# huangzh13/StyleGAN.pytorch

Measured on AMD Instinct MI355X. Metric: img/s full G+D train step, 1024x1024 depth-9 bf16, higher is better.
Workload: dtype bf16; 1 GPU; ffhq1024: StyleGAN 1024x1024, progressive depth index 8, logistic+R1, alpha 0.5, batch 4/GPU, global batch 4; global_batch=4, parallelism=dp1

## Files before the change

### include/sgx.h

```cpp
#ifndef SGX_H
#define SGX_H
#include <stddef.h>
#include <stdint.h>
#ifdef __cplusplus
extern "C" {
#endif

enum { SGX_F32 = 0, SGX_BF16 = 1 };
enum { SGX_ACT_NONE = 0, SGX_ACT_LRELU = 1, SGX_ACT_RELU = 2 };
enum { SGX_EINVAL = -1, SGX_EUNSUPPORTED = -2, SGX_EWORKSPACE = -3 };

int sgx_version(void);
const char* sgx_last_error(void);
int sgx_clear_error(void);
int sgx_stream_wait_stream(void* waiter, void* signaler);
int sgx_selftest_tr16(void* out256, void* stream);

int sgx_prof_start(int mode, int only_of);
int sgx_prof_count(void);
int sgx_prof_get(int i, char* name, int name_cap, float* ms, double* flops, double* bytes, char* desc, int desc_cap);

int sgx_conv3x3(const void* x, const void* w, const float* bias, void* y, int B, int H, int W, int Cin, int Cout,
                int act, const void* mask, int dtype, void* stream);
int sgx_conv4x4s2_down(const void* x, const void* w, const float* bias, void* y, int B, int H, int W, int Cin,
// ... 103 lines not shown
int sgx_rgbconv_pack(const float* w0, float s0, const float* wr, float sr, const float* br, float bscale, void* wf, void* wd, int C,
                     void* stream);
int sgx_rgbconv_fwd(const float* img, const void* wf, const float* b0, void* y, void* bits, int B, int H, int W, int C, int epi, int ones,
                    int dtype, void* stream);
int sgx_rgbconv_tune(int fwd_variant, int nit, int dbg);
int sgx_rgbconv_dgrad(const void* gz, const void* wd, float* gi, int B, int H, int W, int C, int dtype, void* stream);
size_t sgx_rgbconv_wgrad_ws_bytes(int B, int H, int W, int C);
int sgx_rgbconv_wgrad(const float* img, const void* gz, int ones, const float* w0, float s0, const float* wr, float sr, const float* br,
                      float bscale, float* dw0, float* db0, float* dwr, float* dbr, int acc, void* ws, size_t ws_bytes, int B, int H, int W,
                      int C, int dtype, void* stream);
int sgx_blur3x3_stats(const void* x, void* y, const float* bias, const float* noise, const float* nw, double* part,
                      size_t part_bytes, int B, int H, int W, int C, int act, int dtype, void* stream);
int sgx_gepi_bwd(const void* dy, const void* x, const float* bias, const float* noise, const float* nw,
                 const float* style, const float* mean, const float* rstd, void* dx, float* dstyle, float* dnw,
                 float* dbias, void* ws, size_t ws_bytes, int B, int HW, int C, int flags, int dtype, void* stream);

int sgx_pixelnorm_fwd(const float* x, float* y, int B, int C, void* stream);
int sgx_pixelnorm_bwd(const float* dy, const float* x, float* dx, int B, int C, void* stream);
int sgx_mbstd_fwd(const void* x, void* y, int B, int HW, int C, int Cpad, int dtype, void* stream);
int sgx_mbstd_bwd(const void* dy, const void* x, void* dx, int B, int HW, int C, int Cpad, int dtype, void* stream);
int sgx_mbstd_bwd2(const void* ggx, const void* dy, const void* x, void* ddy, void* gx, int B, int HW, int C, int Cpad,
                   int dtype, void* stream);
size_t sgx_sumsq_ws_bytes(void);
int sgx_sumsq_f32(const float* x, size_t n, void* ws, size_t ws_bytes, float* out, void* stream);
int sgx_scale_dev_f32(const float* x, const float* s, float alpha, float* out, size_t n, void* stream);
int sgx_logistic_loss(const float* fake, int n_fake, const float* real, int n_real, float scale, int generator, float* loss,
                      float* g_fake, float* g_real, void* stream);
size_t sgx_gemm_ws_bytes(int M, int N, int K);
int sgx_gemm_f32(const float* A, const float* Bm, float* C, int M, int N, int K, int ta, int tb, float alpha,
                 void* ws, size_t ws_bytes, void* stream);
// ... 34 lines not shown
```

### stylegan/pytorch_amd/Blocks.py

```python
import os

import torch
import torch.nn as nn

from . import functional as F
from .CustomLayers import (BlurLayer, EqualizedConv2d, EqualizedLinear, LayerEpilogue, StddevLayer, View, act_code, apply_act)
from .native import ACT_LRELU, ACT_NONE


FUSE_EPI_STATS = int(os.environ.get("SGX_FUSE_EPI_STATS", "2"))
FUSE_EPI_STATS_MIN = int(os.environ.get("SGX_FUSE_EPI_STATS_MIN", str(1 << 27)))


FUSE_BLUR_BWD = os.environ.get("SGX_FUSE_BLUR_BWD", "1") != "0"


def _lat(d, k):
    return d[k] if isinstance(d, (tuple, list)) else d[:, k]


class InputBlock(nn.Module):

    def __init__(self, nf, dlatent_size, const_input_layer, gain, use_wscale, use_noise, use_pixel_norm,
                 use_instance_norm, use_styles, activation_layer):
# ... 38 lines not shown
        self.conv0_up = EqualizedConv2d(in_channels, out_channels, kernel_size=3, gain=gain, use_wscale=use_wscale,
                                        intermediate=blur, upscale=True)
        self.epi1 = LayerEpilogue(out_channels, dlatent_size, use_wscale, use_noise, use_pixel_norm,
                                  use_instance_norm, use_styles, activation_layer)
        self.conv1 = EqualizedConv2d(out_channels, out_channels, kernel_size=3, gain=gain, use_wscale=use_wscale)
        self.epi2 = LayerEpilogue(out_channels, dlatent_size, use_wscale, use_noise, use_pixel_norm,
                                  use_instance_norm, use_styles, activation_layer)

    def forward_nhwc(self, x, dlatents_in_range, defer_epi2=False):
        up = self.conv0_up
        if (FUSE_EPI_STATS & 1) and self.epi1._fusable and up.intermediate is not None and up.intermediate._is_121:
            b, h, w, _ = x.shape
            nin = self.epi1.noise_inputs((b, 2 * h, 2 * w, up.weight.shape[0]), x.device)
            x, part = up.forward_nhwc(x, skip_bias=True, epi_stats=(up.scaled_bias(),) + nin)
            x = self.epi1.forward_nhwc(x, _lat(dlatents_in_range, 0), conv_bias=up.scaled_bias(), noise_in=nin, pre_stats=part)
        else:
            x = up.forward_nhwc(x, skip_bias=True)
            x = self.epi1.forward_nhwc(x, _lat(dlatents_in_range, 0), conv_bias=up.scaled_bias())
        defer_epi2 = defer_epi2 and self.epi2._fusable
        if (FUSE_EPI_STATS & 2) and self.epi2._fusable and x.numel() >= FUSE_EPI_STATS_MIN:
            nin = self.epi2.noise_inputs(x.shape, x.device)
            x, part = self.conv1.forward_nhwc(x, skip_bias=True, epi_stats=(self.conv1.scaled_bias(),) + nin)
            if defer_epi2:
                return x, (self.conv1.scaled_bias(), nin[0], nin[1], self.epi2._style(_lat(dlatents_in_range, 1)), part)
            return self.epi2.forward_nhwc(x, _lat(dlatents_in_range, 1), conv_bias=self.conv1.scaled_bias(), noise_in=nin, pre_stats=part)
        if defer_epi2:
            nin = self.epi2.noise_inputs(x.shape, x.device)
            x = self.conv1.forward_nhwc(x, skip_bias=True)
            return x, (self.conv1.scaled_bias(), nin[0], nin[1], self.epi2._style(_lat(dlatents_in_range, 1)), None)
        x = self.conv1.forward_nhwc(x, skip_bias=True)
# ... 94 lines not shown
```

### stylegan/pytorch_amd/CustomLayers.py

```python
import math

import numpy as np
import torch
import torch.nn as nn

from . import functional as F
from .native import ACT_LRELU, ACT_NONE, ACT_RELU, EPI_ACT, EPI_NORM

MBSTD_CPAD = 32


def act_code(activation_layer):
    if isinstance(activation_layer, nn.LeakyReLU) and abs(activation_layer.negative_slope - 0.2) < 1e-12:
        return ACT_LRELU
    if activation_layer is torch.relu or isinstance(activation_layer, nn.ReLU):
        return ACT_RELU
    raise NotImplementedError(f"activation {activation_layer!r}: the reference offers 'lrelu' (0.2) and 'relu'")


def apply_act(x, act):
    return F.call(F.BiasActFn, x, None, 1.0, act) if act else x


class PixelNormLayer(nn.Module):
# ... 144 lines not shown
        if bias:
            self.bias = nn.Parameter(torch.zeros(output_channels))
            self.b_mul = lrmul
        else:
            self.bias = None
            self.b_mul = 1
        self.intermediate = intermediate
        assert stride == 1

    def scaled_bias(self):
        if self.bias is None:
            return None
        return self.bias * self.b_mul if self.b_mul != 1 else self.bias

    def forward_nhwc(self, x, act=ACT_NONE, skip_bias=False, out_dtype=None, defer_act=False, x_masked=False, out_scale=1.0,
                     epi_stats=None, x_pre=None, sign_bits=False, x_pre_bits=None, fade=None):
        bias = None if skip_bias else self.scaled_bias()
        cin, cout = self.weight.shape[1], self.weight.shape[0]
        if self.kernel_size == 1:
            assert self.upscale is None and self.downscale is None and self.intermediate is None
            if cin == 3 and x.shape[3] == 3:
                if out_scale != 1.0:
                    y = F.call(F.RgbInFn, x.float(), self.weight, None if bias is None else bias * float(out_scale),
                               self.w_mul * float(out_scale), out_dtype or torch.float32)
                else:
                    y = F.call(F.RgbInFn, x.float(), self.weight, bias, self.w_mul, out_dtype or torch.float32)
            elif cin % 3 == 0 and cin > 3 and x.shape[3] == cin and cout != 3:
                y = None
                for k in range(0, cin, 3):
                    part = F.call(F.RgbInFn, x[..., k:k + 3].float().contiguous(), self.weight[:, k:k + 3].contiguous(),
                                  bias if k == 0 else None, self.w_mul, out_dtype or torch.float32)
# ... 7 lines not shown
        if epi_stats is not None:
            assert skip_bias and act == ACT_NONE and self.downscale is None
            ebias, noise, nw = epi_stats
            if self.upscale is not None:
                fused = min(x.shape[1], x.shape[2]) * 2 >= 128
                y = F.conv(x, self.weight, None, "U" if fused else "UF", self.w_mul)
                assert self.intermediate is not None and self.intermediate._is_121
                return F.call(F.BlurStatsFn, y, ebias, noise, nw)
            assert self.intermediate is None
            if F.conv_stats_nparts(x, self.weight.shape[0]) > 0:
                return F.conv(x, self.weight, None, "S", self.w_mul, ipad=x.shape[3], stats=(ebias, noise, nw))
            return F.conv(x, self.weight, None, "S", self.w_mul, ipad=x.shape[3]), None
        if self.upscale is not None:
            fused = min(x.shape[1], x.shape[2]) * 2 >= 128
            mode = "U" if fused else "UF"
            if (self.intermediate is not None and self.intermediate._is_121
                    and F.conv_blur_ok(x, self.weight.shape[0], mode, False)):
                y = F.call(F.ConvBlurFn, x, self.weight, mode, float(self.w_mul), int(self.weight.shape[1]), False, None)
            else:
                y = F.conv(x, self.weight, None, mode, self.w_mul)
                if self.intermediate is not None:
                    y = self.intermediate.forward_nhwc(y)
            if bias is not None or act:
                y = F.call(F.BiasActFn, y, bias, 1.0, act)
            return y
        if self.downscale is not None:
            assert self.intermediate is None
            if fade is not None:
                assert act == ACT_LRELU and not x_masked
                if x_pre is not None and getattr(x, "_sgx_pre_of", None) is not x_pre:
# ... 77 lines not shown
        self.top_epi = nn.Sequential(OrderedDict(layers))
        self.style_mod = StyleMod(dlatent_size, channels, use_wscale=use_wscale) if use_styles else None
        self._act = act_code(activation_layer)
        self._use = (bool(use_noise), bool(use_pixel_norm), bool(use_instance_norm), bool(use_styles))
        self._fusable = use_noise and use_instance_norm and use_styles and not use_pixel_norm and self._act == ACT_LRELU

    def _style(self, dlatents_in_slice):
        if isinstance(dlatents_in_slice, F.PreStyle):
            return dlatents_in_slice.style
        return self.style_mod.style(dlatents_in_slice)

    def noise_inputs(self, x_shape, device):
        noise_layer = self.top_epi.noise
        return noise_layer.sample(x_shape, device), noise_layer.weight

    def forward_nhwc(self, x, dlatents_in_slice, conv_bias=None, noise_in=None, pre_stats=None):
        use_noise, use_pixel_norm, use_instance_norm, use_styles = self._use
        noise = nw = None
        if noise_in is not None:
            noise, nw = noise_in
        elif use_noise:
            noise, nw = self.noise_inputs(x.shape, x.device)
        style = self._style(dlatents_in_slice) if use_styles else None
        if self._fusable:
            return F.call(F.GEpilogueFn, x, conv_bias, noise, nw, style, EPI_ACT | EPI_NORM, pre_stats)
        assert pre_stats is None
        lrelu = self._act == ACT_LRELU
        norm = EPI_NORM if use_instance_norm else 0
        if lrelu and not use_pixel_norm:
            return F.call(F.GEpilogueFn, x, conv_bias, noise, nw, style, EPI_ACT | norm)
        x = F.call(F.GEpilogueFn, x, conv_bias, noise, nw, None, EPI_ACT if lrelu else 0)
        if not lrelu:
            x = apply_act(x, self._act)
        if use_pixel_norm:
            shape, dt = x.shape, x.dtype
            x = F.call(F.PixelNormFn, x.reshape(-1, shape[3])).reshape(shape).to(dt)
        if norm or style is not None:
            x = F.call(F.GEpilogueFn, x, None, None, None, style, norm)
        return x

    def forward(self, x, dlatents_in_slice=None):
# ... 48 lines not shown
```

### stylegan/pytorch_amd/functional.py

```python
import contextlib
import functools
import os
import weakref

import numpy as np
import torch
from torch.autograd import Function
from torch.autograd.function import once_differentiable

from . import native as N

_DATA_GRAD_ONLY = 0


@contextlib.contextmanager
def data_grad_only():
    global _DATA_GRAD_ONLY
    _DATA_GRAD_ONLY += 1
    try:
        yield
    finally:
        _DATA_GRAD_ONLY -= 1


# ... 1545 lines not shown
        x, bias_c, noise, nw_c, style_c, mean, rstd = ctx.saved_tensors
        gy = _c(gy)
        B, H, W, C = x.shape
        dx = torch.empty_like(x)
        dstyle = torch.empty((B, 2 * C), dtype=torch.float32, device=x.device)
        dnw = torch.empty((C,), dtype=torch.float32, device=x.device)
        dbias = torch.empty((C,), dtype=torch.float32, device=x.device) if ctx.has_bias else None
        L = N.lib()
        ws = N.workspace(L.sgx_gepi_ws_bytes(B, H * W, C), x.device)
        N.check(L.sgx_gepi_bwd(N.ptr(gy), N.ptr(x), N.ptr(bias_c), N.ptr(noise), N.ptr(nw_c), N.ptr(style_c), N.ptr(mean), N.ptr(rstd),
                               N.ptr(dx), N.ptr(dstyle), N.ptr(dnw), N.ptr(dbias), N.ptr(ws), ws.numel(), B, H * W, C, ctx.flags,
                               N.dt(x), N.stream()), "sgx_gepi_bwd")
        return dx, dbias, None, dnw if ctx.has_noise else None, dstyle if ctx.has_style else None, None, None


FUSE_EPI_RGB = os.environ.get("SGX_FUSE_EPI_RGB", "1") != "0"


def epi_rgb_out_ok(C, dtype):
    ve = 4 if dtype == torch.float32 else 8
    if dtype not in (torch.float32, torch.bfloat16) or C % ve or C > 2048:
        return False
    lpp = min(C // ve, 16)
    return lpp & (lpp - 1) == 0


class EpiRgbOutFn(Function):

    @staticmethod
    def forward(ctx, y, ebias, noise, nw, style, weight, rbias, wscale, low, alpha, pre=None):
# ... 521 lines not shown
```

### stylegan/pytorch_amd/native.py

```python
import ctypes
import os
import subprocess
import threading

import torch

_HERE = os.path.dirname(os.path.abspath(__file__))
LIB_PATH = os.environ.get("SGX_HIP_LIB") or os.path.join(_HERE, "libsgx_hip.so")
CSRC = os.path.join(_HERE, "csrc")

F32, BF16 = 0, 1
ACT_NONE, ACT_LRELU, ACT_RELU = 0, 1, 2
EPI_ACT, EPI_NORM = 1, 2
PACK_S, PACK_D, PACK_U, PACK_UF = 0, 1, 2, 3

_lib = None
_lock = threading.Lock()

c_void_p, c_int, c_float, c_size_t = ctypes.c_void_p, ctypes.c_int, ctypes.c_float, ctypes.c_size_t
P, I, F, Z = c_void_p, c_int, c_float, c_size_t

SIGNATURES = {
    "sgx_version": (I, []),
    "sgx_last_error": (ctypes.c_char_p, []),
# ... 65 lines not shown
    "sgx_conv4x4s2_up_blur": (I, [P, P, P, P, I, I, I, I, I, I, P]),
    "sgx_conv4x4s2_up_blur_bits": (I, [P, P, P, P, I, I, I, I, I, I, P]),
    "sgx_pack_upblur": (I, [P, P, I, I, I, I, F, P]),
    "sgx_conv_upblur_ok": (I, [I, I, I, I, I, I]),
    "sgx_conv_upblur": (I, [P, P, P, P, I, I, I, I, I, I, P]),
    "sgx_rgbconv_ok": (I, [I, I, I, I, I]),
    "sgx_rgbconv_pack": (I, [P, F, P, F, P, F, P, P, I, P]),
    "sgx_rgbconv_fwd": (I, [P, P, P, P, P, I, I, I, I, I, I, I, P]),
    "sgx_rgbconv_tune": (I, [I, I, I]),
    "sgx_rgbconv_dgrad": (I, [P, P, P, I, I, I, I, I, P]),
    "sgx_rgbconv_wgrad_ws_bytes": (Z, [I, I, I, I]),
    "sgx_rgbconv_wgrad": (I, [P, P, I, P, F, P, F, P, F, P, P, P, P, I, P, Z, I, I, I, I, I, P]),
    "sgx_conv3x3_stats": (I, [P, P, P, P, P, P, P, Z, I, I, I, I, I, I, P]),
    "sgx_blur3x3_stats": (I, [P, P, P, P, P, P, Z, I, I, I, I, I, I, P]),
    "sgx_gepi_bwd": (I, [P, P, P, P, P, P, P, P, P, P, P, P, P, Z, I, I, I, I, I, P]),
    "sgx_pixelnorm_fwd": (I, [P, P, I, I, P]),
    "sgx_pixelnorm_bwd": (I, [P, P, P, I, I, P]),
    "sgx_mbstd_fwd": (I, [P, P, I, I, I, I, I, P]),
    "sgx_mbstd_bwd": (I, [P, P, P, I, I, I, I, I, P]),
    "sgx_mbstd_bwd2": (I, [P, P, P, P, P, I, I, I, I, I, P]),
    "sgx_sumsq_ws_bytes": (Z, []),
    "sgx_sumsq_f32": (I, [P, Z, P, Z, P, P]),
    "sgx_scale_dev_f32": (I, [P, P, F, P, Z, P]),
    "sgx_logistic_loss": (I, [P, I, P, I, F, I, P, P, P, P]),
    "sgx_gemm_ws_bytes": (Z, [I, I, I]),
    "sgx_gemm_f32": (I, [P, P, P, I, I, I, I, I, F, P, Z, P]),
    "sgx_linear_fwd": (I, [P, P, P, P, I, I, I, F, F, I, P]),
    "sgx_linear_bwd_data": (I, [P, P, P, P, I, I, I, F, P]),
    "sgx_linear_bwd_param": (I, [P, P, P, P, P, I, I, I, F, F, P]),
    "sgx_style_fwd": (I, [P, P, P, I, I, I, I, P]),
# ... 217 lines not shown
```

Baseline: 290.1 img/s.

## Fuse blur, noise, bias, lrelu, instance norm and style into single-pass generator layer kernel

Adds a fused generator-layer kernel (forward and backward) for small and mid-resolution layers. It keeps each per-channel-group image slice resident in registers or LDS, computes the instance-norm statistics in-block, and applies the epilogue without a second pass over memory. For upsample layers where the conv+blur fused path is unavailable, the blur is folded into the same kernel. The backward uses ticket-based last-block reduction for the noise-weight and bias gradients, which saves a separate finish launch but adds atomics and a persistent ticket buffer.

```diff
diff --git a/include/sgx.h b/include/sgx.h
--- a/include/sgx.h
+++ b/include/sgx.h
@@ -141,6 +141,12 @@
 int sgx_gepi_bwd(const void* dy, const void* x, const float* bias, const float* noise, const float* nw,
                  const float* style, const float* mean, const float* rstd, void* dx, float* dstyle, float* dnw,
                  float* dbias, void* ws, size_t ws_bytes, int B, int HW, int C, int flags, int dtype, void* stream);
+int sgx_glayer_ok(int B, int H, int W, int C, int flags, int dtype);
+int sgx_glayer_fwd(const void* x, int blur, const float* bias, const float* noise, const float* nw, const float* style, void* xb, void* y,
+                   float* mean, float* rstd, int B, int H, int W, int C, int flags, int dtype, void* stream);
+int sgx_glayer_bwd(const void* dy, const void* xb, int blur, const float* bias, const float* noise, const float* nw, const float* style,
+                   const float* mean, const float* rstd, void* dx, float* dstyle, float* dnw, float* dbias, double* part, int* tickets,
+                   int B, int H, int W, int C, int flags, int dtype, void* stream);
 
 int sgx_pixelnorm_fwd(const float* x, float* y, int B, int C, void* stream);
 int sgx_pixelnorm_bwd(const float* dy, const float* x, float* dx, int B, int C, void* stream);
diff --git a/stylegan/pytorch_amd/Blocks.py b/stylegan/pytorch_amd/Blocks.py
--- a/stylegan/pytorch_amd/Blocks.py
+++ b/stylegan/pytorch_amd/Blocks.py
@@ -76,6 +76,11 @@
             nin = self.epi1.noise_inputs((b, 2 * h, 2 * w, up.weight.shape[0]), x.device)
             x, part = up.forward_nhwc(x, skip_bias=True, epi_stats=(up.scaled_bias(),) + nin)
             x = self.epi1.forward_nhwc(x, _lat(dlatents_in_range, 0), conv_bias=up.scaled_bias(), noise_in=nin, pre_stats=part)
+        elif (up.intermediate is not None and up.intermediate._is_121
+              and self.epi1.glayer_takes((x.shape[0], 2 * x.shape[1], 2 * x.shape[2], up.weight.shape[0]), x.dtype)
+              and not F.conv_blur_ok(x, up.weight.shape[0], "U" if min(x.shape[1], x.shape[2]) * 2 >= 128 else "UF", False)):
+            x = up.forward_nhwc(x, skip_bias=True, skip_blur=True)
+            x = self.epi1.forward_nhwc(x, _lat(dlatents_in_range, 0), conv_bias=up.scaled_bias(), blur=True)
         else:
             x = up.forward_nhwc(x, skip_bias=True)
             x = self.epi1.forward_nhwc(x, _lat(dlatents_in_range, 0), conv_bias=up.scaled_bias())
diff --git a/stylegan/pytorch_amd/CustomLayers.py b/stylegan/pytorch_amd/CustomLayers.py
--- a/stylegan/pytorch_amd/CustomLayers.py
+++ b/stylegan/pytorch_amd/CustomLayers.py
@@ -182,7 +182,7 @@
         return self.bias * self.b_mul if self.b_mul != 1 else self.bias
 
     def forward_nhwc(self, x, act=ACT_NONE, skip_bias=False, out_dtype=None, defer_act=False, x_masked=False, out_scale=1.0,
-                     epi_stats=None, x_pre=None, sign_bits=False, x_pre_bits=None, fade=None):
+                     epi_stats=None, x_pre=None, sign_bits=False, x_pre_bits=None, fade=None, skip_blur=False):
         bias = None if skip_bias else self.scaled_bias()
         cin, cout = self.weight.shape[1], self.weight.shape[0]
         if self.kernel_size == 1:
@@ -220,6 +220,9 @@
         if self.upscale is not None:
             fused = min(x.shape[1], x.shape[2]) * 2 >= 128
             mode = "U" if fused else "UF"
+            if skip_blur:
+                assert skip_bias and not act and self.intermediate is not None and self.intermediate._is_121
+                return F.conv(x, self.weight, None, mode, self.w_mul)
             if (self.intermediate is not None and self.intermediate._is_121
                     and F.conv_blur_ok(x, self.weight.shape[0], mode, False)):
                 y = F.call(F.ConvBlurFn, x, self.weight, mode, float(self.w_mul), int(self.weight.shape[1]), False, None)
@@ -327,7 +330,10 @@
         noise_layer = self.top_epi.noise
         return noise_layer.sample(x_shape, device), noise_layer.weight
 
-    def forward_nhwc(self, x, dlatents_in_slice, conv_bias=None, noise_in=None, pre_stats=None):
+    def glayer_takes(self, x_shape, dtype):
+        return bool(self._fusable and F.glayer_ok(x_shape, dtype))
+
+    def forward_nhwc(self, x, dlatents_in_slice, conv_bias=None, noise_in=None, pre_stats=None, blur=False):
         use_noise, use_pixel_norm, use_instance_norm, use_styles = self._use
         noise = nw = None
         if noise_in is not None:
@@ -336,8 +342,11 @@
             noise, nw = self.noise_inputs(x.shape, x.device)
         style = self._style(dlatents_in_slice) if use_styles else None
         if self._fusable:
+            if pre_stats is None and F.glayer_ok(x.shape, x.dtype):
+                return F.call(F.GLayerFn, x, conv_bias, noise, nw, style, blur)
+            assert not blur
             return F.call(F.GEpilogueFn, x, conv_bias, noise, nw, style, EPI_ACT | EPI_NORM, pre_stats)
-        assert pre_stats is None
+        assert pre_stats is None and not blur
         lrelu = self._act == ACT_LRELU
         norm = EPI_NORM if use_instance_norm else 0
         if lrelu and not use_pixel_norm:
diff --git a/stylegan/pytorch_amd/csrc/gepi_layer.hip b/stylegan/pytorch_amd/csrc/gepi_layer.hip
--- /dev/null
+++ b/stylegan/pytorch_amd/csrc/gepi_layer.hip
@@ -0,0 +1,633 @@
+#include "common.h"
+
+#define GL_EPS 1e-5f
+#define GL_CG 16
+#define GL_VE 8
+#define GL_NV (GL_CG / GL_VE)
+#define GL_W2 (2 * GL_VE)
+
+__device__ __forceinline__ void gl_coef(const float* __restrict__ p, float (&k)[GL_VE]) {
+#pragma unroll
+    for (int j = 0; j < GL_VE; j += 4) {
+        const float4 t = *reinterpret_cast<const float4*>(p + j);
+        k[j] = t.x; k[j + 1] = t.y; k[j + 2] = t.z; k[j + 3] = t.w;
+    }
+}
+__device__ __forceinline__ void gl_unpack(const uint4& q, float (&v)[GL_VE]) {
+    const unsigned w[4] = {q.x, q.y, q.z, q.w};
+#pragma unroll
+    for (int i = 0; i < 4; ++i) { v[2 * i] = __uint_as_float(w[i] << 16); v[2 * i + 1] = __uint_as_float(w[i] & 0xffff0000u); }
+}
+__device__ __forceinline__ uint4 gl_pack(const float (&v)[GL_VE]) {
+    return make_uint4(pack_bf16x2(v[0], v[1]), pack_bf16x2(v[2], v[3]), pack_bf16x2(v[4], v[5]), pack_bf16x2(v[6], v[7]));
+}
+
+template <int NT>
+__device__ __forceinline__ void gl_block_sum(const float (&q0)[GL_VE], const float (&q1)[GL_VE], double* sh, double* tot) {
+    constexpr int NWV = NT / 64;
+    const int t = threadIdx.x, lane = t & 63, wv = t >> 6;
+#pragma unroll
+    for (int j = 0; j < GL_W2; ++j) {
+        double d = (double)(j < GL_VE ? q0[j < GL_VE ? j : 0] : q1[j < GL_VE ? 0 : j - GL_VE]);
+#pragma unroll
+        for (int o = 32; o >= GL_NV; o >>= 1) d += __shfl_xor(d, o, 64);
+        if (lane < GL_NV) sh[(wv * GL_NV + lane) * GL_W2 + j] = d;
+    }
+    __syncthreads();
+    if (t < GL_NV * GL_W2) {
+        const int v = t / GL_W2, j = t % GL_W2;
+        double a = 0.0;
+#pragma unroll
+        for (int w = 0; w < NWV; ++w) a += sh[(w * GL_NV + v) * GL_W2 + j];
+        tot[t] = a;
+    }
+    __syncthreads();
+}
+
+__device__ __forceinline__ uint4 gl_blur(const uint4* tile, int p, int v, int H, int W) {
+    const int h = p / W, w = p - h * W;
+    const bool hasl = w > 0, hasr = w + 1 < W;
+    float hs[3][GL_VE];
+#pragma unroll
+    for (int k = 0; k < 3; ++k) {
+        const int r = h - 1 + k;
+        if ((unsigned)r < (unsigned)H) {
+            const int q = r * W + w;
+            float l[GL_VE], m[GL_VE], rr[GL_VE];
+            gl_unpack(tile[q * GL_NV + v], m);
+            gl_unpack(tile[(hasl ? q - 1 : q) * GL_NV + v], l);
+            gl_unpack(tile[(hasr ? q + 1 : q) * GL_NV + v], rr);
+#pragma unroll
+            for (int j = 0; j < GL_VE; ++j) hs[k][j] = (hasl ? l[j] : 0.f) + 2.f * m[j] + (hasr ? rr[j] : 0.f);
+        } else {
+#pragma unroll
+            for (int j = 0; j < GL_VE; ++j) hs[k][j] = 0.f;
+        }
+    }
+    float o[GL_VE];
+#pragma unroll
+    for (int j = 0; j < GL_VE; ++j) o[j] = (hs[0][j] + 2.f * hs[1][j] + hs[2][j]) * (1.f / 16.f);
+    return gl_pack(o);
+}
+
+template <int NT, int IT, bool BLUR>
+__global__ __launch_bounds__(NT) void glayer_fwd_kernel(const bf16_t* __restrict__ x, const float* __restrict__ bias, const float* __restrict__ noise,
+                                                        const float* __restrict__ nw, const float* __restrict__ style, bf16_t* __restrict__ xbo,
+                                                        bf16_t* __restrict__ y, float* __restrict__ mean_out, float* __restrict__ rstd_out, int H, int W,
+                                                        int C) {
+    constexpr int R = NT / GL_NV;
+    __shared__ double sh[(NT / 64) * GL_NV * GL_W2 + 32];
+    __shared__ float sstat[2 * GL_CG];
+    __shared__ uint4 tile[BLUR ? IT * NT : 1];
+    double* const tot = sh + (NT / 64) * GL_NV * GL_W2;
+    const int b = blockIdx.y, t = threadIdx.x, v = t % GL_NV, r = t / GL_NV, HW = H * W;
+    const int cv = C / GL_VE, vg = blockIdx.x * GL_NV + v, c0 = vg * GL_VE;
+    float kb[GL_VE], kw[GL_VE], s0[GL_VE], s1[GL_VE];
+#pragma unroll
+    for (int j = 0; j < GL_VE; ++j) { kb[j] = 0.f; s0[j] = 0.f; s1[j] = 0.f; }
+    if (bias) gl_coef(bias + c0, kb);
+    gl_coef(nw + c0, kw);
+    const size_t base = ((size_t)b * HW * cv + vg) * GL_VE;
+    const float* nzb = noise + (size_t)b * HW;
+    uint4 xq[IT];
+    float nz[IT];
+#pragma unroll
+    for (int i = 0; i < IT; ++i) {
+        const int p = r + i * R;
+        const bool ok = p < HW;
+        const uint4 xl = *reinterpret_cast<const uint4*>(x + base + (size_t)(ok ? p : 0) * cv * GL_VE);
+        const float nl = nzb[ok ? p : 0];
+        xq[i] = make_uint4(ok ? xl.x : 0u, ok ? xl.y : 0u, ok ? xl.z : 0u, ok ? xl.w : 0u);
+        nz[i] = ok ? nl : 0.f;
+    }
+    if (BLUR) {
+#pragma unroll
+        for (int i = 0; i < IT; ++i) {
+            const int p = r + i * R;
+            if (p < HW) tile[p * GL_NV + v] = xq[i];
+        }
+        __syncthreads();
+#pragma unroll
+        for (int i = 0; i < IT; ++i) {
+            const int p = r + i * R;
+            if (p < HW) {
+                xq[i] = gl_blur(tile, p, v, H, W);
+                *reinterpret_cast<uint4*>(xbo + base + (size_t)p * cv * GL_VE) = xq[i];
+            }
+        }
+    }
+#pragma unroll
+    for (int i = 0; i < IT; ++i) {
+        if (r + i * R < HW) {
+            float xv[GL_VE];
+            gl_unpack(xq[i], xv);
+#pragma unroll
+            for (int j = 0; j < GL_VE; ++j) {
+                const float a = act_apply(xv[j] + kb[j] + kw[j] * nz[i], SGX_ACT_LRELU);
+                s0[j] += a; s1[j] += a * a;
+            }
+        }
+    }
+    gl_block_sum<NT>(s0, s1, sh, tot);
+    if (t < GL_CG) {
+        const int vv = t / GL_VE, j = t % GL_VE;
+        const double mm = tot[vv * GL_W2 + j] / HW;
+        double var = tot[vv * GL_W2 + GL_VE + j] / HW - mm * mm;
+        if (var < 0.0) var = 0.0;
+        const float m = (float)mm, rs = (float)(1.0 / sqrt(var + (double)GL_EPS));
+        sstat[t] = m; sstat[GL_CG + t] = rs;
+        mean_out[(size_t)b * C + blockIdx.x * GL_CG + t] = m;
+        rstd_out[(size_t)b * C + blockIdx.x * GL_CG + t] = rs;
+    }
+    __syncthreads();
+    float km[GL_VE], kr[GL_VE], ks[GL_VE], k1[GL_VE];
+#pragma unroll
+    for (int j = 0; j < GL_VE; ++j) { km[j] = sstat[v * GL_VE + j]; kr[j] = sstat[GL_CG + v * GL_VE + j]; }
+    gl_coef(style + (size_t)b * 2 * C + c0, ks);
+    gl_coef(style + (size_t)b * 2 * C + C + c0, k1);
+#pragma unroll
+    for (int j = 0; j < GL_VE; ++j) ks[j] += 1.f;
+#pragma unroll
+    for (int i = 0; i < IT; ++i) {
+        const int p = r + i * R;
+        if (p < HW) {
+            float xv[GL_VE];
+            gl_unpack(xq[i], xv);
+#pragma unroll
+            for (int j = 0; j < GL_VE; ++j) {
+                const float a = act_apply(xv[j] + kb[j] + kw[j] * nz[i], SGX_ACT_LRELU);
+                const float xh = (a - km[j]) * kr[j];
+                xv[j] = xh * ks[j] + k1[j];
+            }
+            *reinterpret_cast<uint4*>(y + base + (size_t)p * cv * GL_VE) = gl_pack(xv);
+        }
+    }
+}
+
+template <bool COHERENT>
+__device__ __forceinline__ void gl_finish(const double* part, float* __restrict__ dnw, float* __restrict__ dbias, int nrows, int C, int cbase,
+                                          int nch, int nwaves) {
+    const int lane = threadIdx.x & 63, wv = threadIdx.x >> 6;
+    for (int ci = wv; ci < nch; ci += nwaves) {
+        const int c = cbase + ci;
+        double a = 0.0, d = 0.0;
+        for (int k = lane; k < nrows; k += 64) {
+            const double* p = part + ((size_t)k * C + c) * 2;
+            if (COHERENT) {
+                a += __longlong_as_double((long long)__hip_atomic_load(reinterpret_cast<const unsigned long long*>(p), __ATOMIC_RELAXED, __HIP_MEMORY_SCOPE_AGENT));
+                d += __longlong_as_double((long long)__hip_atomic_load(reinterpret_cast<const unsigned long long*>(p + 1), __ATOMIC_RELAXED, __HIP_MEMORY_SCOPE_AGENT));
+            } else {
+                const double2 q = *reinterpret_cast<const double2*>(p);
+                a += q.x; d += q.y;
+            }
+        }
+        a = wave_sum_d(a); d = wave_sum_d(d);
+        if (lane == 0) {
+            dnw[c] = (float)a;
+            if (dbias) dbias[c] = (float)d;
+        }
+    }
+}
+
+__device__ __forceinline__ void gl_part_store(double* o, double a0, double a1, bool through) {
+    if (through) {
+        __hip_atomic_store(reinterpret_cast<unsigned long long*>(o), (unsigned long long)__double_as_longlong(a0), __ATOMIC_RELAXED, __HIP_MEMORY_SCOPE_AGENT);
+        __hip_atomic_store(reinterpret_cast<unsigned long long*>(o + 1), (unsigned long long)__double_as_longlong(a1), __ATOMIC_RELAXED, __HIP_MEMORY_SCOPE_AGENT);
+    } else {
+        o[0] = a0; o[1] = a1;
+    }
+}
+__device__ __forceinline__ void gl_ticket_finish(const double* part, float* __restrict__ dnw, float* __restrict__ dbias, int* tickets, int* last,
+                                                 int nrows, int C, int nwaves) {
+    asm volatile("s_waitcnt vmcnt(0)" ::: "memory");
+    __syncthreads();
+    if (threadIdx.x == 0) *last = __hip_atomic_fetch_add(tickets + blockIdx.x, 1, __ATOMIC_RELAXED, __HIP_MEMORY_SCOPE_AGENT) == (int)gridDim.y - 1;
+    __syncthreads();
+    if (!*last) return;
+    gl_finish<true>(part, dnw, dbias, nrows, C, blockIdx.x * GL_CG, GL_CG, nwaves);
+    if (threadIdx.x == 0) __hip_atomic_store(tickets + blockIdx.x, 0, __ATOMIC_RELAXED, __HIP_MEMORY_SCOPE_AGENT);
+}
+
+template <int NT, int IT, bool BLUR>
+__global__ __launch_bounds__(NT) void glayer_bwd_kernel(const bf16_t* __restrict__ x, const bf16_t* __restrict__ dy, bf16_t* __restrict__ dx,
+                                                        const float* __restrict__ bias, const float* __restrict__ noise, const float* __restrict__ nw,
+                                                        const float* __restrict__ style, const float* __restrict__ mean, const float* __restrict__ rstd,
+                                                        float* __restrict__ dstyle, double* part, float* __restrict__ dnw, float* __restrict__ dbias,
+                                                        int* tickets, int H, int W, int C) {
+    constexpr int R = NT / GL_NV;
+    __shared__ double sh[(NT / 64) * GL_NV * GL_W2 + 32];
+    __shared__ float scoef[2 * GL_CG];
+    __shared__ uint4 tile[BLUR ? IT * NT : 1];
+    double* const tot = sh + (NT / 64) * GL_NV * GL_W2;
+    const int b = blockIdx.y, t = threadIdx.x, v = t % GL_NV, r = t / GL_NV, HW = H * W;
+    const int cv = C / GL_VE, vg = blockIdx.x * GL_NV + v, c0 = vg * GL_VE;
+    float kb[GL_VE], kw[GL_VE], km[GL_VE], kr[GL_VE], ks[GL_VE], s0[GL_VE], s1[GL_VE];
+#pragma unroll
+    for (int j = 0; j < GL_VE; ++j) { kb[j] = 0.f; s0[j] = 0.f; s1[j] = 0.f; }
+    if (bias) gl_coef(bias + c0, kb);
+    gl_coef(nw + c0, kw);
+    gl_coef(mean + (size_t)b * C + c0, km);
+    gl_coef(rstd + (size_t)b * C + c0, kr);
+    gl_coef(style + (size_t)b * 2 * C + c0, ks);
+#pragma unroll
+    for (int j = 0; j < GL_VE; ++j) ks[j] += 1.f;
+    const size_t base = ((size_t)b * HW * cv + vg) * GL_VE;
+    const float* nzb = noise + (size_t)b * HW;
+    uint4 xq[IT], gq[IT];
+    float nz[IT];
+#pragma unroll
+    for (int i = 0; i < IT; ++i) {
+        const int p = r + i * R;
+        const bool ok = p < HW;
+        const size_t po = (size_t)(ok ? p : 0) * cv * GL_VE;
+        const uint4 xl = *reinterpret_cast<const uint4*>(x + base + po), gl = *reinterpret_cast<const uint4*>(dy + base + po);
+        const float nl = nzb[ok ? p : 0];
+        xq[i] = make_uint4(ok ? xl.x : 0u, ok ? xl.y : 0u, ok ? xl.z : 0u, ok ? xl.w : 0u);
+        gq[i] = make_uint4(ok ? gl.x : 0u, ok ? gl.y : 0u, ok ? gl.z : 0u, ok ? gl.w : 0u);
+        nz[i] = ok ? nl : 0.f;
+    }
+#pragma unroll
+    for (int i = 0; i < IT; ++i) {
+        if (r + i * R < HW) {
+            float xv[GL_VE], gv[GL_VE];
+            gl_unpack(xq[i], xv); gl_unpack(gq[i], gv);
+#pragma unroll
+            for (int j = 0; j < GL_VE; ++j) {
+                const float xh = (act_apply(xv[j] + kb[j] + kw[j] * nz[i], SGX_ACT_LRELU) - km[j]) * kr[j];
+                s0[j] += gv[j]; s1[j] += gv[j] * xh;
+            }
+        }
+    }
+    gl_block_sum<NT>(s0, s1, sh, tot);
+    if (t < GL_CG) {
+        const int vv = t / GL_VE, j = t % GL_VE, c = blockIdx.x * GL_CG + t;
+        const double sdy = tot[vv * GL_W2 + j], sdx = tot[vv * GL_W2 + GL_VE + j];
+        if (dstyle) {
+            dstyle[(size_t)b * 2 * C + c] = (float)sdx;
+            dstyle[(size_t)b * 2 * C + C + c] = (float)sdy;
+        }
+        const double sc = (double)style[(size_t)b * 2 * C + c] + 1.0;
+        scoef[t] = (float)(sc * sdy / HW);
+        scoef[GL_CG + t] = (float)(sc * sdx / HW);
+    }
+    __syncthreads();
+    float k1[GL_VE], k2[GL_VE];
+#pragma unroll
+    for (int j = 0; j < GL_VE; ++j) { k1[j] = scoef[v * GL_VE + j]; k2[j] = scoef[GL_CG + v * GL_VE + j]; s0[j] = 0.f; s1[j] = 0.f; }
+#pragma unroll
+    for (int i = 0; i < IT; ++i) {
+        const int p = r + i * R;
+        if (p < HW) {
+            float xv[GL_VE], gv[GL_VE], ov[GL_VE];
+            gl_unpack(xq[i], xv); gl_unpack(gq[i], gv);
+#pragma unroll
+            for (int j = 0; j < GL_VE; ++j) {
+                const float pp = xv[j] + kb[j] + kw[j] * nz[i];
+                const float xh = (act_apply(pp, SGX_ACT_LRELU) - km[j]) * kr[j];
+                const float da = kr[j] * (gv[j] * ks[j] - k1[j] - xh * k2[j]);
+                const float dp = da * lrelu_slope(pp);
+                ov[j] = dp;
+                s0[j] += dp * nz[i]; s1[j] += dp;
+            }
+            const uint4 o = gl_pack(ov);
+            if (BLUR) tile[p * GL_NV + v] = o;
+            else *reinterpret_cast<uint4*>(dx + base + (size_t)p * cv * GL_VE) = o;
+        }
+    }
+    gl_block_sum<NT>(s0, s1, sh, tot);
+    if (t < GL_CG) {
+        const int vv = t / GL_VE, j = t % GL_VE;
+        gl_part_store(part + ((size_t)b * C + blockIdx.x * GL_CG + t) * 2, tot[vv * GL_W2 + j], tot[vv * GL_W2 + GL_VE + j], tickets != nullptr);
+    }
+    if (BLUR) {
+#pragma unroll
+        for (int i = 0; i < IT; ++i) {
+            const int p = r + i * R;
+            if (p < HW) *reinterpret_cast<uint4*>(dx + base + (size_t)p * cv * GL_VE) = gl_blur(tile, p, v, H, W);
+        }
+    }
+    if (!tickets) return;
+    gl_ticket_finish(part, dnw, dbias, tickets, reinterpret_cast<int*>(sh), (int)gridDim.y, C, NT / 64);
+}
+
+__global__ __launch_bounds__(256) void glayer_fin_kernel(const double* part, float* __restrict__ dnw, float* __restrict__ dbias, int nrows, int C) {
+    const int cbase = blockIdx.x * 4, nch = C - cbase < 4 ? C - cbase : 4;
+    gl_finish<false>(part, dnw, dbias, nrows, C, cbase, nch, 4);
+}
+
+#define GL_LNT 1024
+#define GL_STRIP 8
+
+struct GlGeom { int rows, rpt, chunk, nchunk, L; };
+
+template <typename Fetch, typename Put>
+__device__ __forceinline__ void gl_blur_strips(int H, int W, Fetch fetch, Put put) {
+    const int strips = (H + GL_STRIP - 1) / GL_STRIP, n = strips * W * GL_NV;
+    for (int u = threadIdx.x; u < n; u += GL_LNT) {
+        const int v = u % GL_NV, q = u / GL_NV, w = q % W, h0 = (q / W) * GL_STRIP;
+        const bool hasl = w > 0, hasr = w + 1 < W;
+        float ha[GL_VE], hb[GL_VE], hc[GL_VE];
+#pragma unroll
+        for (int j = 0; j < GL_VE; ++j) { ha[j] = 0.f; hb[j] = 0.f; }
+#pragma unroll
+        for (int k = 0; k < GL_STRIP + 2; ++k) {
+            const int r = h0 - 1 + k;
+            if ((unsigned)r < (unsigned)H) {
+                float l[GL_VE], m[GL_VE], rr[GL_VE];
+                gl_unpack(fetch(r, w, v), m);
+                gl_unpack(fetch(r, hasl ? w - 1 : w, v), l);
+                gl_unpack(fetch(r, hasr ? w + 1 : w, v), rr);
+#pragma unroll
+                for (int j = 0; j < GL_VE; ++j) hc[j] = (hasl ? l[j] : 0.f) + 2.f * m[j] + (hasr ? rr[j] : 0.f);
+            } else {
+#pragma unroll
+                for (int j = 0; j < GL_VE; ++j) hc[j] = 0.f;
+            }
+            if (k >= 2 && r - 1 < H) {
+                float o[GL_VE];
+#pragma unroll
+                for (int j = 0; j < GL_VE; ++j) o[j] = (ha[j] + 2.f * hb[j] + hc[j]) * (1.f / 16.f);
+                put(r - 1, w, v, gl_pack(o));
+            }
+#pragma unroll
+            for (int j = 0; j < GL_VE; ++j) { ha[j] = hb[j]; hb[j] = hc[j]; }
+        }
+    }
+}
+
+__device__ __forceinline__ void gl_chunk_totals(const double* l2, int c16, int nchunk, int L, double& A0, double& A1) {
+    A0 = 0.0; A1 = 0.0;
+    for (int l = 0; l < L; ++l) {
+        double t0 = 0.0, t1 = 0.0;
+        for (int k = l; k < nchunk; k += L) { t0 += l2[(k * GL_CG + c16) * 2]; t1 += l2[(k * GL_CG + c16) * 2 + 1]; }
+        A0 += t0; A1 += t1;
+    }
+}
+
+template <bool BLUR>
+__global__ __launch_bounds__(GL_LNT) void glayer_lds_fwd_kernel(const bf16_t* __restrict__ x, const float* __restrict__ bias, const float* __restrict__ noise,
+                                                                const float* __restrict__ nw, const float* __restrict__ style, bf16_t* __restrict__ xbo,
+                                                                bf16_t* __restrict__ y, float* __restrict__ mean_out, float* __restrict__ rstd_out, int H,
+                                                                int W, int C, GlGeom g) {
+    extern __shared__ uint4 gl_lds[];
+    const int HW = H * W, b = blockIdx.y, t = threadIdx.x;
+    uint4* const tile = gl_lds;
+    double* const l2 = reinterpret_cast<double*>(tile + (size_t)HW * GL_NV);
+    float* const sstat = reinterpret_cast<float*>(l2 + (size_t)g.nchunk * GL_CG * 2);
+    const int cb = blockIdx.x * GL_CG;
+    const size_t base = (size_t)b * HW * C + cb;
+    const float* nzb = noise + (size_t)b * HW;
+    if (BLUR) {
+        gl_blur_strips(H, W, [&](int r, int w, int v) { return *reinterpret_cast<const uint4*>(x + base + (size_t)(r * W + w) * C + v * GL_VE); },
+                       [&](int r, int w, int v, const uint4& o) {
+                           tile[(r * W + w) * GL_NV + v] = o;
+                           *reinterpret_cast<uint4*>(xbo + base + (size_t)(r * W + w) * C + v * GL_VE) = o;
+                       });
+    } else {
+        for (int i = t; i < HW * GL_NV; i += GL_LNT)
+            tile[i] = *reinterpret_cast<const uint4*>(x + base + (size_t)(i / GL_NV) * C + (i % GL_NV) * GL_VE);
+    }
+    __syncthreads();
+    const bf16_t* const tl = reinterpret_cast<const bf16_t*>(tile);
+    for (int o = t; o < g.nchunk * GL_CG; o += GL_LNT) {
+        const int ch = o / GL_CG, c = o % GL_CG;
+        const float kb = bias ? bias[cb + c] : 0.f, kw = nw[cb + c];
+        const int p0 = ch * g.chunk, p1 = p0 + g.chunk < HW ? p0 + g.chunk : HW;
+        double a0 = 0.0, a1 = 0.0;
+        for (int tr = 0; tr < g.rows; ++tr) {
+            float s0 = 0.f, s1 = 0.f;
+#pragma unroll 8
+            for (int p = p0 + tr; p < p1; p += g.rows) {
+                const float a = act_apply(bf2f(tl[p * GL_CG + c]) + kb + kw * nzb[p], SGX_ACT_LRELU);
+                s0 += a; s1 += a * a;
+            }
+            a0 += (double)s0; a1 += (double)s1;
+        }
+        l2[o * 2] = a0; l2[o * 2 + 1] = a1;
+    }
+    __syncthreads();
+    if (t < GL_CG) {
+        double sum, sq;
+        gl_chunk_totals(l2, t, g.nchunk, g.L, sum, sq);
+        const double mm = sum / HW;
+        double var = sq / HW - mm * mm;
+        if (var < 0.0) var = 0.0;
+        const float m = (float)mm, rs = (float)(1.0 / sqrt(var + (double)GL_EPS));
+        sstat[t] = m; sstat[GL_CG + t] = rs;
+        mean_out[(size_t)b * C + cb + t] = m;
+        rstd_out[(size_t)b * C + cb + t] = rs;
+    }
+    __syncthreads();
+    const int v = t % GL_NV, c0 = cb + v * GL_VE;
+    float kb[GL_VE], kw[GL_VE], km[GL_VE], kr[GL_VE], ks[GL_VE], k1[GL_VE];
+#pragma unroll
+    for (int j = 0; j < GL_VE; ++j) { kb[j] = 0.f; km[j] = sstat[v * GL_VE + j]; kr[j] = sstat[GL_CG + v * GL_VE + j]; }
+    if (bias) gl_coef(bias + c0, kb);
+    gl_coef(nw + c0, kw);
+    gl_coef(style + (size_t)b * 2 * C + c0, ks);
+    gl_coef(style + (size_t)b * 2 * C + C + c0, k1);
+#pragma unroll
+    for (int j = 0; j < GL_VE; ++j) ks[j] += 1.f;
+#pragma unroll 4
+    for (int i = t; i < HW * GL_NV; i += GL_LNT) {
+        const int p = i / GL_NV;
+        const float nz = nzb[p];
+        float xv[GL_VE];
+        gl_unpack(tile[i], xv);
+#pragma unroll
+        for (int j = 0; j < GL_VE; ++j) {
+            const float a = act_apply(xv[j] + kb[j] + kw[j] * nz, SGX_ACT_LRELU);
+            const float xh = (a - km[j]) * kr[j];
+            xv[j] = xh * ks[j] + k1[j];
+        }
+        *reinterpret_cast<uint4*>(y + base + (size_t)p * C + v * GL_VE) = gl_pack(xv);
+    }
+}
+
+template <bool BLUR>
+__global__ __launch_bounds__(GL_LNT) void glayer_lds_bwd_kernel(const bf16_t* __restrict__ x, const bf16_t* __restrict__ dy, bf16_t* __restrict__ dx,
+                                                                const float* __restrict__ bias, const float* __restrict__ noise, const float* __restrict__ nw,
+                                                                const float* __restrict__ style, const float* __restrict__ mean, const float* __restrict__ rstd,
+                                                                float* __restrict__ dstyle, double* part, float* __restrict__ dnw, float* __restrict__ dbias,
+                                                                int* tickets, int H, int W, int C, GlGeom g) {
+    extern __shared__ uint4 gl_lds[];
+    const int HW = H * W, b = blockIdx.y, t = threadIdx.x;
+    uint4* const tile = gl_lds;
+    double* const l2 = reinterpret_cast<double*>(tile + (size_t)HW * GL_NV);
+    float* const scoef = reinterpret_cast<float*>(l2 + (size_t)g.nchunk * GL_CG * 2);
+    const int cb = blockIdx.x * GL_CG;
+    const size_t base = (size_t)b * HW * C + cb;
+    const float* nzb = noise + (size_t)b * HW;
+    for (int i = t; i < HW * GL_NV; i += GL_LNT)
+        tile[i] = *reinterpret_cast<const uint4*>(x + base + (size_t)(i / GL_NV) * C + (i % GL_NV) * GL_VE);
+    __syncthreads();
+    bf16_t* const tl = reinterpret_cast<bf16_t*>(tile);
+    for (int o = t; o < g.nchunk * GL_CG; o += GL_LNT) {
+        const int ch = o / GL_CG, c = o % GL_CG;
+        const float kb = bias ? bias[cb + c] : 0.f, kw = nw[cb + c], km = mean[(size_t)b * C + cb + c], kr = rstd[(size_t)b * C + cb + c];
+        const int p0 = ch * g.chunk, p1 = p0 + g.chunk < HW ? p0 + g.chunk : HW;
+        double a0 = 0.0, a1 = 0.0;
+        for (int tr = 0; tr < g.rows; ++tr) {
+            float s0 = 0.f, s1 = 0.f;
+#pragma unroll 8
+            for (int p = p0 + tr; p < p1; p += g.rows) {
+                const float gv = bf2f(dy[base + (size_t)p * C + c]);
+                const float xh = (act_apply(bf2f(tl[p * GL_CG + c]) + kb + kw * nzb[p], SGX_ACT_LRELU) - km) * kr;
+                s0 += gv; s1 += gv * xh;
+            }
+            a0 += (double)s0; a1 += (double)s1;
+        }
+        l2[o * 2] = a0; l2[o * 2 + 1] = a1;
+    }
+    __syncthreads();
+    if (t < GL_CG) {
+        double sdy, sdx;
+        gl_chunk_totals(l2, t, g.nchunk, g.L, sdy, sdx);
+        const int c = cb + t;
+        if (dstyle) {
+            dstyle[(size_t)b * 2 * C + c] = (float)sdx;
+            dstyle[(size_t)b * 2 * C + C + c] = (float)sdy;
+        }
+        const double sc = (double)style[(size_t)b * 2 * C + c] + 1.0;
+        scoef[t] = (float)(sc * sdy / HW);
+        scoef[GL_CG + t] = (float)(sc * sdx / HW);
+    }
+    __syncthreads();
+    for (int o = t; o < g.nchunk * GL_CG; o += GL_LNT) {
+        const int ch = o / GL_CG, c = o % GL_CG;
+        const float kb = bias ? bias[cb + c] : 0.f, kw = nw[cb + c], km = mean[(size_t)b * C + cb + c], kr = rstd[(size_t)b * C + cb + c];
+        const float ks = style[(size_t)b * 2 * C + cb + c] + 1.f, k1 = scoef[c], k2 = scoef[GL_CG + c];
+        const int p0 = ch * g.chunk, p1 = p0 + g.chunk < HW ? p0 + g.chunk : HW;
+        double a0 = 0.0, a1 = 0.0;
+        for (int tr = 0; tr < g.rows; ++tr) {
+            float s0 = 0.f, s1 = 0.f;
+#pragma unroll 8
+            for (int p = p0 + tr; p < p1; p += g.rows) {
+                const float gv = bf2f(dy[base + (size_t)p * C + c]), nz = nzb[p];
+                const float pp = bf2f(tl[p * GL_CG + c]) + kb + kw * nz;
+                const float xh = (act_apply(pp, SGX_ACT_LRELU) - km) * kr;
+                const float da = kr * (gv * ks - k1 - xh * k2);
+                const float dp = da * lrelu_slope(pp);
+                tl[p * GL_CG + c] = (bf16_t)(pack_bf16x2(dp, 0.f) & 0xffffu);
+                s0 += dp * nz; s1 += dp;
+            }
+            a0 += (double)s0; a1 += (double)s1;
+        }
+        gl_part_store(part + (((size_t)b * g.nchunk + ch) * C + cb + c) * 2, a0, a1, tickets != nullptr);
+    }
+    __syncthreads();
+    if (BLUR) {
+        gl_blur_strips(H, W, [&](int r, int w, int v) { return tile[(r * W + w) * GL_NV + v]; },
+                       [&](int r, int w, int v, const uint4& o) { *reinterpret_cast<uint4*>(dx + base + (size_t)(r * W + w) * C + v * GL_VE) = o; });
+    } else {
+        for (int i = t; i < HW * GL_NV; i += GL_LNT)
+            *reinterpret_cast<uint4*>(dx + base + (size_t)(i / GL_NV) * C + (i % GL_NV) * GL_VE) = tile[i];
+    }
+    if (!tickets) return;
+    gl_ticket_finish(part, dnw, dbias, tickets, reinterpret_cast<int*>(l2), (int)gridDim.y * g.nchunk, C, GL_LNT / 64);
+}
+
+static GlGeom gl_geom(int B, int HW, int C) {
+    GlGeom g;
+    const int cvt = C / GL_VE;
+    g.rows = 256 / cvt;
+    static const int rpt_max = [] { const char* e = getenv("SGX_GEPI_RPT"); const int v = e ? atoi(e) : 0; return v > 0 ? v : 64; }();
+    g.rpt = rpt_max;
+    while (g.rpt > 8 && (long)B * ((HW + g.rows * g.rpt - 1) / (g.rows * g.rpt)) < 512) g.rpt >>= 1;
+    g.chunk = g.rows * g.rpt;
+    g.nchunk = (HW + g.chunk - 1) / g.chunk;
+    g.L = 256 / (C < 256 ? C : 256);
+    return g;
+}
+#define GL_LDS_MAX (160 * 1024)
+static size_t gl_lds_bytes(int HW, const GlGeom& g) { return (size_t)HW * GL_NV * 16 + (size_t)g.nchunk * GL_CG * 2 * sizeof(double) + 2 * GL_CG * sizeof(float); }
+
+static int gl_plan(int HW) { return HW <= 2 * (256 / GL_NV) ? 0 : (HW <= 1024 ? 1 : 2); }
+
+SGX_SWITCH(gl_lds_on, "SGX_GLAYER_LDS", 0)
+static int gl_can(int B, int H, int W, int C, int flags, int dtype) {
+    if (dtype != SGX_BF16 || flags != (SGX_EPI_ACT | SGX_EPI_NORM)) return 0;
+    if (B < 1 || H < 1 || W < 1 || C < GL_CG || C % GL_CG != 0) return 0;
+    const long HW = (long)H * W, bytes = (long)B * HW * C * 2;
+    if ((long)B * (C / GL_CG) < 64 || HW > 4096) return 0;
+    if (HW > 256 && bytes > (8L << 20)) return 0;
+    if (HW > 1024) {
+        const int cv = C / GL_VE;
+        if (C < 128 || cv > 256 || (cv & (cv - 1)) != 0) return 0;
+        if (gl_lds_bytes((int)HW, gl_geom(B, (int)HW, C)) > GL_LDS_MAX) return 0;
+    }
+    return C / GL_CG;
+}
+extern "C" int sgx_glayer_ok(int B, int H, int W, int C, int flags, int dtype) {
+    if ((long)H * W > 1024 && !gl_lds_on()) return 0;
+    return gl_can(B, H, W, C, flags, dtype);
+}
+
+extern "C" int sgx_glayer_fwd(const void* x, int blur, const float* bias, const float* noise, const float* nw, const float* style, void* xb,
+                              void* y, float* mean, float* rstd, int B, int H, int W, int C, int flags, int dtype, void* stream) {
+    hipStream_t st = (hipStream_t)stream;
+    SGX_REQUIRE(gl_can(B, H, W, C, flags, dtype), SGX_EUNSUPPORTED, "glayer_fwd: B=%d %dx%d C=%d flags=%d dtype=%d has no plan",
+                B, H, W, C, flags, dtype);
+    SGX_REQUIRE(x && noise && nw && style && y && mean && rstd && (!blur || xb), SGX_EINVAL, "glayer_fwd: null argument");
+    const dim3 grid(C / GL_CG, B);
+    const bf16_t* xp = (const bf16_t*)x;
+    bf16_t *xo = (bf16_t*)xb, *yp = (bf16_t*)y;
+    SGX_NOTE(0.0, (blur ? 6.0 : 4.0) * B * H * W * C, "glayer_fwd B%d HW%d C%d blur%d", B, H * W, C, blur ? 1 : 0);
+    if (gl_plan(H * W) == 2) {
+        const GlGeom g = gl_geom(B, H * W, C);
+        const size_t lds = gl_lds_bytes(H * W, g);
+        if (blur) {
+            sgx_lds_opt_in<glayer_lds_fwd_kernel<true>>(GL_LDS_MAX);
+            hipLaunchKernelGGL(glayer_lds_fwd_kernel<true>, grid, dim3(GL_LNT), lds, st, xp, bias, noise, nw, style, xo, yp, mean, rstd, H, W, C, g);
+        } else {
+            sgx_lds_opt_in<glayer_lds_fwd_kernel<false>>(GL_LDS_MAX);
+            hipLaunchKernelGGL(glayer_lds_fwd_kernel<false>, grid, dim3(GL_LNT), lds, st, xp, bias, noise, nw, style, xo, yp, mean, rstd, H, W, C, g);
+        }
+    } else if (gl_plan(H * W) == 0) {
+        if (blur) hipLaunchKernelGGL((glayer_fwd_kernel<256, 2, true>), grid, dim3(256), 0, st, xp, bias, noise, nw, style, xo, yp, mean, rstd, H, W, C);
+        else hipLaunchKernelGGL((glayer_fwd_kernel<256, 2, false>), grid, dim3(256), 0, st, xp, bias, noise, nw, style, xo, yp, mean, rstd, H, W, C);
+    } else {
+        if (blur) hipLaunchKernelGGL((glayer_fwd_kernel<512, 4, true>), grid, dim3(512), 0, st, xp, bias, noise, nw, style, xo, yp, mean, rstd, H, W, C);
+        else hipLaunchKernelGGL((glayer_fwd_kernel<512, 4, false>), grid, dim3(512), 0, st, xp, bias, noise, nw, style, xo, yp, mean, rstd, H, W, C);
+    }
+    SGX_LAUNCH_CHECK("glayer_fwd");
+    return 0;
+}
+
+extern "C" int sgx_glayer_bwd(const void* dy, const void* xb, int blur, const float* bias, const float* noise, const float* nw, const float* style,
+                              const float* mean, const float* rstd, void* dx, float* dstyle, float* dnw, float* dbias, double* part, int* tickets,
+                              int B, int H, int W, int C, int flags, int dtype, void* stream) {
+    hipStream_t st = (hipStream_t)stream;
+    SGX_REQUIRE(gl_can(B, H, W, C, flags, dtype), SGX_EUNSUPPORTED, "glayer_bwd: B=%d %dx%d C=%d flags=%d dtype=%d has no plan",
+                B, H, W, C, flags, dtype);
+    SGX_REQUIRE(dy && xb && noise && nw && style && mean && rstd && dx && dnw && part, SGX_EINVAL, "glayer_bwd: null argument");
+    const dim3 grid(C / GL_CG, B);
+    const bf16_t *xp = (const bf16_t*)xb, *gp = (const bf16_t*)dy;
+    bf16_t* dp = (bf16_t*)dx;
+    SGX_NOTE(0.0, 6.0 * B * H * W * C, "glayer_bwd B%d HW%d C%d blur%d", B, H * W, C, blur ? 1 : 0);
+    int nrows = B;
+    if (gl_plan(H * W) == 2) {
+        const GlGeom g = gl_geom(B, H * W, C);
+        const size_t lds = gl_lds_bytes(H * W, g);
+        nrows = B * g.nchunk;
+        if (blur) {
+            sgx_lds_opt_in<glayer_lds_bwd_kernel<true>>(GL_LDS_MAX);
+            hipLaunchKernelGGL(glayer_lds_bwd_kernel<true>, grid, dim3(GL_LNT), lds, st, xp, gp, dp, bias, noise, nw, style, mean, rstd, dstyle, part, dnw, dbias, tickets, H, W, C, g);
+        } else {
+            sgx_lds_opt_in<glayer_lds_bwd_kernel<false>>(GL_LDS_MAX);
+            hipLaunchKernelGGL(glayer_lds_bwd_kernel<false>, grid, dim3(GL_LNT), lds, st, xp, gp, dp, bias, noise, nw, style, mean, rstd, dstyle, part, dnw, dbias, tickets, H, W, C, g);
+        }
+    } else if (gl_plan(H * W) == 0) {
+        if (blur) hipLaunchKernelGGL((glayer_bwd_kernel<256, 2, true>), grid, dim3(256), 0, st, xp, gp, dp, bias, noise, nw, style, mean, rstd, dstyle, part, dnw, dbias, tickets, H, W, C);
+        else hipLaunchKernelGGL((glayer_bwd_kernel<256, 2, false>), grid, dim3(256), 0, st, xp, gp, dp, bias, noise, nw, style, mean, rstd, dstyle, part, dnw, dbias, tickets, H, W, C);
+    } else {
+        if (blur) hipLaunchKernelGGL((glayer_bwd_kernel<512, 4, true>), grid, dim3(512), 0, st, xp, gp, dp, bias, noise, nw, style, mean, rstd, dstyle, part, dnw, dbias, tickets, H, W, C);
+        else hipLaunchKernelGGL((glayer_bwd_kernel<512, 4, false>), grid, dim3(512), 0, st, xp, gp, dp, bias, noise, nw, style, mean, rstd, dstyle, part, dnw, dbias, tickets, H, W, C);
+    }
+    SGX_LAUNCH_CHECK("glayer_bwd");
+    if (!tickets) {
+        hipLaunchKernelGGL(glayer_fin_kernel, dim3((C + 3) / 4), dim3(256), 0, st, (const double*)part, dnw, dbias, nrows, C);
+        SGX_LAUNCH_CHECK("glayer_fin");
+    }
+    return 0;
+}
diff --git a/stylegan/pytorch_amd/functional.py b/stylegan/pytorch_amd/functional.py
--- a/stylegan/pytorch_amd/functional.py
+++ b/stylegan/pytorch_amd/functional.py
@@ -1583,6 +1583,70 @@
         return dx, dbias, None, dnw if ctx.has_noise else None, dstyle if ctx.has_style else None, None, None
 
 
+GLAYER = os.environ.get("SGX_GLAYER", "1") != "0"
+_GLAYER_TICKETS = {}
+_GLAYER_TICKETS_N = 256
+
+
+def glayer_ok(shape, dtype, flags=N.EPI_ACT | N.EPI_NORM):
+    if not GLAYER or dtype != torch.bfloat16:
+        return 0
+    B, H, W, C = shape
+    return int(N.lib().sgx_glayer_ok(int(B), int(H), int(W), int(C), int(flags), N.BF16))
+
+
+def _glayer_tickets(device, need):
+    if need > _GLAYER_TICKETS_N:
+        return None
+    key = (device.index, N.stream())
+    t = _GLAYER_TICKETS.get(key)
+    if t is None:
+        if N.capturing():
+            return None
+        t = _GLAYER_TICKETS[key] = torch.zeros(_GLAYER_TICKETS_N, dtype=torch.int32, device=device)
+    return t
+
+
+class GLayerFn(Function):
+
+    @staticmethod
+    def forward(ctx, x, bias, noise, nw, style, blur=False):
+        x = _c(x)
+        B, H, W, C = x.shape
+        noise = _c(noise.detach().reshape(B, H * W))
+        if noise.dtype != torch.float32:
+            noise = noise.float()
+        nw_c, style_c = _c(nw.detach()), _c(style.detach())
+        bias_c = None if bias is None else _c(bias.detach())
+        xb = torch.empty_like(x) if blur else None
+        y = torch.empty_like(x)
+        mean = torch.empty((B, C), dtype=torch.float32, device=x.device)
+        rstd = torch.empty_like(mean)
+        N.check(N.lib().sgx_glayer_fwd(N.ptr(x), int(bool(blur)), N.ptr(bias_c), N.ptr(noise), N.ptr(nw_c), N.ptr(style_c), N.ptr(xb), N.ptr(y),
+                                       N.ptr(mean), N.ptr(rstd), B, H, W, C, N.EPI_ACT | N.EPI_NORM, N.dt(x), N.stream()), "sgx_glayer_fwd")
+        ctx.has_bias, ctx.blur = bias is not None, bool(blur)
+        ctx.save_for_backward(xb if blur else x, bias_c, noise, nw_c, style_c, mean, rstd)
+        return y
+
+    @staticmethod
+    @once_differentiable
+    def backward(ctx, gy):
+        xb, bias_c, noise, nw_c, style_c, mean, rstd = ctx.saved_tensors
+        gy = _c(gy)
+        B, H, W, C = xb.shape
+        dx = torch.empty_like(xb)
+        dstyle = torch.empty((B, 2 * C), dtype=torch.float32, device=xb.device)
+        dnw = torch.empty((C,), dtype=torch.float32, device=xb.device)
+        dbias = torch.empty((C,), dtype=torch.float32, device=xb.device) if ctx.has_bias else None
+        L = N.lib()
+        part = N.workspace(L.sgx_gepi_ws_bytes(B, H * W, C), xb.device)
+        tickets = _glayer_tickets(xb.device, C // 16)
+        N.check(L.sgx_glayer_bwd(N.ptr(gy), N.ptr(xb), int(ctx.blur), N.ptr(bias_c), N.ptr(noise), N.ptr(nw_c), N.ptr(style_c), N.ptr(mean),
+                                 N.ptr(rstd), N.ptr(dx), N.ptr(dstyle), N.ptr(dnw), N.ptr(dbias), N.ptr(part), N.ptr(tickets), B, H, W, C,
+                                 N.EPI_ACT | N.EPI_NORM, N.dt(xb), N.stream()), "sgx_glayer_bwd")
+        return dx, dbias, None, dnw, dstyle, None
+
+
 FUSE_EPI_RGB = os.environ.get("SGX_FUSE_EPI_RGB", "1") != "0"
 
 
diff --git a/stylegan/pytorch_amd/native.py b/stylegan/pytorch_amd/native.py
--- a/stylegan/pytorch_amd/native.py
+++ b/stylegan/pytorch_amd/native.py
@@ -103,6 +103,9 @@
     "sgx_conv3x3_stats": (I, [P, P, P, P, P, P, P, Z, I, I, I, I, I, I, P]),
     "sgx_blur3x3_stats": (I, [P, P, P, P, P, P, Z, I, I, I, I, I, I, P]),
     "sgx_gepi_bwd": (I, [P, P, P, P, P, P, P, P, P, P, P, P, P, Z, I, I, I, I, I, P]),
+    "sgx_glayer_ok": (I, [I, I, I, I, I, I]),
+    "sgx_glayer_fwd": (I, [P, I, P, P, P, P, P, P, P, P, I, I, I, I, I, I, P]),
+    "sgx_glayer_bwd": (I, [P, P, I, P, P, P, P, P, P, P, P, P, P, P, P, I, I, I, I, I, I, P]),
     "sgx_pixelnorm_fwd": (I, [P, P, I, I, P]),
     "sgx_pixelnorm_bwd": (I, [P, P, P, I, I, P]),
     "sgx_mbstd_fwd": (I, [P, P, I, I, I, I, I, P]),
```

Result: no change. 291.2 img/s (median of 6 runs) (+0.4%).
